# cmavro/GNN-RAG

Measured on NVIDIA H100. Metric: questions/sec (GNN forward+score) on WebQSP-shape subgraphs; agg-kernel HBM GB/s, higher is better.
Workload: dtype f32

## Files before the change

### gnn_rag_b200/csrc/linear_tc.cu

```cuda
#include "wgmma.cuh"

namespace gr {

int g_tc_cluster = 1;
int g_tc_bk = 32;
int g_tc_tma_store = 1;

namespace {

using namespace tc;
constexpr int kThreads = 384;
constexpr int kConsumerWarps = 8;
constexpr int kLaunchRegs = 168, kProducerRegs = 40, kConsumerRegs = 232;
static_assert(128 * kProducerRegs + 256 * kConsumerRegs <= kThreads * kLaunchRegs, "register budget");

__global__ void split_bf16_seg_kernel(const float* __restrict__ W, int64_t ldw, int64_t N, int64_t Kpad,
                                      int seg, int pitch, __nv_bfloat16* __restrict__ hi,
                                      __nv_bfloat16* __restrict__ lo, int64_t ldo) {
  const int64_t total = N * Kpad;
  const int64_t stride = (int64_t)gridDim.x * blockDim.x;
  for (int64_t i = (int64_t)blockIdx.x * blockDim.x + threadIdx.x; i < total; i += stride) {
    const int64_t n = i / Kpad, k = i - n * Kpad;
    const int sidx = (int)(k / pitch), c = (int)(k - (int64_t)sidx * pitch);
    float v = c < seg ? __ldg(W + n * ldw + (int64_t)sidx * seg + c) : 0.f;
// ... 14 lines not shown
    float v[4] = {0.f, 0.f, 0.f, 0.f};
    const float* src = A + m * lda + k;
    if (vec_ok && k + 3 < K) {
      float4 t = __ldg(reinterpret_cast<const float4*>(src));
      v[0] = t.x; v[1] = t.y; v[2] = t.z; v[3] = t.w;
    } else {
#pragma unroll
      for (int q = 0; q < 4; ++q)
        if (k + q < K) v[q] = __ldg(src + q);
    }
    __nv_bfloat16 h[4], l[4];
#pragma unroll
    for (int q = 0; q < 4; ++q) {
      h[q] = __float2bfloat16_rn(v[q]);
      l[q] = __float2bfloat16_rn(v[q] - __bfloat162float(h[q]));
    }
    __nv_bfloat16* ph = hi + m * ldo + k;
    __nv_bfloat16* pl = lo + m * ldo + k;
    if (vec_st && k + 3 < ldo) {
      *reinterpret_cast<uint2*>(ph) = *reinterpret_cast<uint2*>(h);
      *reinterpret_cast<uint2*>(pl) = *reinterpret_cast<uint2*>(l);
    } else {
#pragma unroll
      for (int q = 0; q < 4; ++q)
        if (k + q < ldo) { ph[q] = h[q]; pl[q] = l[q]; }
    }
  }
}

struct TcParams {
  const float* bias;
  float* C;
  int64_t ldc;
  __nv_bfloat16* c_hi;
  __nv_bfloat16* c_lo;
  int64_t ldc16;
  const float* w_score;
  float* dots;
  int M, N, K, n_pad, n16, stages, num_tiles;
  uint32_t flags;
  int tma_store;
  int kg_T, kg_G, kg_pitch, kg_nkb, kg_one0, kg_one1, kg_nb0;
};

template <int NP, int CS, int BK, bool GROUPED>
__global__ void __launch_bounds__(kThreads, 1)
linear_tc_kernel(const __grid_constant__ CUtensorMap map_a_hi, const __grid_constant__ CUtensorMap map_a_lo,
                 const __grid_constant__ CUtensorMap map_w_hi, const __grid_constant__ CUtensorMap map_w_lo,
                 const __grid_constant__ CUtensorMap map_c, const __grid_constant__ CUtensorMap map_c_hi,
                 const __grid_constant__ CUtensorMap map_c_lo, const TcParams p) {
  extern __shared__ __align__(1024) uint8_t smem_raw[];
  uint8_t* smem = reinterpret_cast<uint8_t*>((reinterpret_cast<uintptr_t>(smem_raw) + 1023) & ~(uintptr_t)1023);
  const int a_bytes = BM * BK * 2;
  constexpr int w_bytes = NP * BK * 2;
  const bool single = (p.flags & GR_LINEAR_BF16_SINGLE) != 0;
  const int w_off = single ? a_bytes : 2 * a_bytes;
  const int stage_bytes = single ? a_bytes + w_bytes : 2 * a_bytes + 2 * w_bytes;
  uint8_t* s_out = smem + (size_t)p.stages * stage_bytes;
  uint64_t* bars = reinterpret_cast<uint64_t*>(s_out + 2 * kStageOutBytes);
  uint64_t* full_bar = bars;
  uint64_t* empty_bar = bars + p.stages;
  float* s_bias = reinterpret_cast<float*>(bars + 2 * p.stages);
  float* s_ws = s_bias + 256;
  for (int i = threadIdx.x; i < 256; i += kThreads) {
    s_bias[i] = (p.bias && i < p.N) ? p.bias[i] : 0.f;
    s_ws[i] = (p.w_score && i < p.N) ? p.w_score[i] : 0.f;
// ... 67 lines not shown
    const bool vec_h = p.c_hi && (p.ldc16 % 2 == 0) && ((reinterpret_cast<uintptr_t>(p.c_hi) & 3) == 0) &&
                       ((reinterpret_cast<uintptr_t>(p.c_lo) & 3) == 0);
    uint32_t phase = 0;
    int s = 0;
    for (int g = cid; g < ngroups; g += ncluster) {
      const int tile = g * CS + crank;
      float acc[NP / 2];
#pragma unroll
      for (int i = 0; i < NP / 2; ++i) acc[i] = 0.f;
      int prev = -1;
      for (int kb = 0; kb < nkb; ++kb) {
        mbar_wait(&full_bar[s], phase);
        const uint32_t sa = smem_u32(smem + (size_t)s * stage_bytes);
        const uint32_t a_row = (uint32_t)(cw * WG_M * BK * 2);
        const uint64_t da_hi = make_smem_desc<BK>(sa + a_row), da_lo = make_smem_desc<BK>(sa + a_bytes + a_row);
        const uint64_t dw_hi = make_smem_desc<BK>(sa + w_off), dw_lo = make_smem_desc<BK>(sa + w_off + w_bytes);
        if constexpr (GROUPED) {
          if (kb >= p.kg_one0 && kb < p.kg_one1) mma_kblock<NP, BK, 1, false>(acc, da_hi, da_lo, dw_hi, dw_lo);
          else mma_kblock<NP, BK, BK / MMA_K, false>(acc, da_hi, da_lo, dw_hi, dw_lo);
        } else if (single) {
          mma_kblock<NP, BK, BK / MMA_K, true>(acc, da_hi, da_lo, dw_hi, dw_lo);
        } else {
          mma_kblock<NP, BK, BK / MMA_K, false>(acc, da_hi, da_lo, dw_hi, dw_lo);
        }
        wgmma_wait<1>();
        if (prev >= 0 && lane == 0) release_slot<CS>(&empty_bar[prev]);
        prev = s;
        if (++s == p.stages) { s = 0; phase ^= 1; }
      }
      wgmma_wait<0>();
      if (prev >= 0 && lane == 0) release_slot<CS>(&empty_bar[prev]);

      const int64_t row0 = (int64_t)tile * BM + cw * WG_M + r;
      float dot0 = 0.f, dot1 = 0.f;
#pragma unroll
      for (int q = 0; q < NP / 16; ++q) {
        const int c0 = 16 * q;
        if (c0 >= p.n_pad) continue;
        float v[8];
        epi_values(acc, q, cq, e, v, dot0, dot1);
        if (p.tma_store) {
          epi_store_tma(v, stg, r, cq, issuer, 1 + cw, &map_c, &map_c_hi, &map_c_lo, p.C != nullptr,
                        p.c_hi != nullptr, c0, tile * BM + cw * WG_M);
          continue;
        }
#pragma unroll
        for (int b = 0; b < 2; ++b) {
          const int col = c0 + 8 * b + 2 * cq;
#pragma unroll
          for (int hr = 0; hr < 2; ++hr) {
            const int64_t row = row0 + 8 * hr;
            if (row >= p.M) continue;
            const float x0 = v[4 * b + 2 * hr], x1 = v[4 * b + 2 * hr + 1];
            if (p.C) {
              float* c = p.C + row * p.ldc + col;
              if (vec_c && col + 1 < p.N) {
                *reinterpret_cast<float2*>(c) = make_float2(x0, x1);
              } else {
                if (col < p.N) c[0] = x0;
                if (col + 1 < p.N) c[1] = x1;
              }
            }
            if (p.c_hi) {
              uint32_t lo;
              const uint32_t hi = split_hi_lo(x0, x1, lo);
              unsigned short* ph = reinterpret_cast<unsigned short*>(p.c_hi + row * p.ldc16 + col);
              unsigned short* pl = reinterpret_cast<unsigned short*>(p.c_lo + row * p.ldc16 + col);
              if (vec_h && col + 1 < p.n16) {
                *reinterpret_cast<uint32_t*>(ph) = hi;
                *reinterpret_cast<uint32_t*>(pl) = lo;
              } else {
                if (col < p.n16) { ph[0] = (unsigned short)(hi & 0xFFFF); pl[0] = (unsigned short)(lo & 0xFFFF); }
                if (col + 1 < p.n16) { ph[1] = (unsigned short)(hi >> 16); pl[1] = (unsigned short)(lo >> 16); }
              }
            }
          }
        }
      }
      epi_dots(dot0, dot1, p.dots, row0, p.M, cq);
    }
    if (p.tma_store && issuer) asm volatile("cp.async.bulk.wait_group 0;" ::: "memory");
  }
  __syncthreads();
  if (CS > 1) cluster_sync_all();
}

struct TcPlan {
  int64_t kp;
  int n_pad, np, stages, bk;
  size_t a_plane_bytes, w_plane_bytes, total_bytes, w_only_bytes, smem_bytes;
  bool ok;
};

TcPlan plan_tc(int64_t M, int64_t N, int64_t K, bool single = false) {
  TcPlan t{};
  const int BK = g_tc_bk == 64 ? 64 : 32;
// ... 117 lines not shown
                            void* workspace, size_t workspace_bytes, void* stream_) {
  using namespace gr;
  cudaStream_t stream = reinterpret_cast<cudaStream_t>(stream_);
  GR_CHECK_ARG(A && W && C && workspace, "null pointer");
  GR_CHECK_ARG(M > 0 && N > 0 && K > 0, "M, N, K must be positive");
  GR_CHECK_ARG(lda >= K && ldw >= K && ldc >= N, "leading dimension smaller than row length");
  GR_CHECK_ARG(M < (int64_t)0x7fffffff - BM, "M exceeds int32 range");
  TcPlan t = plan_tc(M, N, K);
  if (!t.ok) {
    set_error("gr_linear_tc: unsupported shape M=%lld N=%lld K=%lld (need 8 <= N <= 256, K >= 8)",
              (long long)M, (long long)N, (long long)K);
    return GR_ERR_UNSUPPORTED;
  }
  if (int rc = check_workspace(__func__, workspace, workspace_bytes, t.total_bytes)) return rc;
  if ((reinterpret_cast<uintptr_t>(workspace) & 255) != 0) {
    set_error("gr_linear_tc: workspace must be 256-byte aligned");
    return GR_ERR_INVALID_ARG;
  }
  char* ws = reinterpret_cast<char*>(workspace);
  __nv_bfloat16* a_hi = reinterpret_cast<__nv_bfloat16*>(ws);
  __nv_bfloat16* a_lo = reinterpret_cast<__nv_bfloat16*>(ws + t.a_plane_bytes);
  __nv_bfloat16* w_hi = reinterpret_cast<__nv_bfloat16*>(ws + 2 * t.a_plane_bytes);
  __nv_bfloat16* w_lo = reinterpret_cast<__nv_bfloat16*>(ws + 2 * t.a_plane_bytes + t.w_plane_bytes);
  int rc = split_launch(A, lda, M, K, a_hi, a_lo, t.kp, stream);
  if (rc != GR_OK) return rc;
  rc = split_launch(W, ldw, N, K, w_hi, w_lo, t.kp, stream);
  if (rc != GR_OK) return rc;
  TcParams p{};
  p.bias = bias; p.C = C; p.ldc = ldc;
  p.M = (int)M; p.N = (int)N; p.K = (int)K; p.flags = flags;
  return launch_tc(a_hi, a_lo, t.kp, w_hi, w_lo, t.kp, t, p, stream);
}

extern "C" int gr_linear_tc_planes(const void* A_hi, const void* A_lo, int64_t lda16, const float* W,
                                   int64_t ldw, const float* bias, float* C, int64_t ldc, void* C_hi,
                                   void* C_lo, int64_t ldc16, const float* w_score, float* dots, int64_t M,
                                   int64_t N, int64_t K, int64_t k_seg, int64_t k_seg_pitch, uint32_t flags,
                                   void* workspace, size_t workspace_bytes, void* stream_) {
  using namespace gr;
  cudaStream_t stream = reinterpret_cast<cudaStream_t>(stream_);
  GR_CHECK_ARG(A_hi && (A_lo || (flags & GR_LINEAR_BF16_SINGLE)) && W && workspace, "null pointer");
  GR_CHECK_ARG(C || C_hi, "no output requested");
  GR_CHECK_ARG(M > 0 && N > 0 && K > 0, "M, N, K must be positive");
  const bool grouped = (flags & GR_LINEAR_K_GROUPED) != 0;
  const bool korder = (flags & GR_LINEAR_K_ORDER_PLANES) != 0;
  GR_CHECK_ARG(!korder || grouped, "GR_LINEAR_K_ORDER_PLANES modifies GR_LINEAR_K_GROUPED and needs it");
  if (grouped) {
    GR_CHECK_ARG(k_seg > 0 && k_seg_pitch >= k_seg && k_seg_pitch % 16 == 0,
                 "GR_LINEAR_K_GROUPED needs segmented K: k_seg > 0 and k_seg_pitch >= k_seg, a multiple of 16");
    GR_CHECK_ARG(K % k_seg_pitch == 0 && (K / k_seg_pitch) % 2 == 1,
                 "GR_LINEAR_K_GROUPED needs an odd number of segments (2 I + 1)");
    GR_CHECK_ARG(g_tc_bk != 64, "GR_LINEAR_K_GROUPED needs 32-column k-blocks (tc_bk = 32)");
    GR_CHECK_ARG(!(flags & GR_LINEAR_BF16_SINGLE), "GR_LINEAR_K_GROUPED does not combine with GR_LINEAR_BF16_SINGLE");
  }
  const bool segmented = grouped || (k_seg > 0 && k_seg_pitch > k_seg);
  GR_CHECK_ARG(lda16 >= K && lda16 % 8 == 0, "lda16 must be >= K and a multiple of 8");
  GR_CHECK_ARG(!segmented || K % k_seg_pitch == 0, "K must be a multiple of k_seg_pitch");
  GR_CHECK_ARG(ldw >= (segmented ? K / k_seg_pitch * k_seg : K), "ldw smaller than the weight row length");
  GR_CHECK_ARG(!C || ldc >= N, "ldc smaller than N");
  GR_CHECK_ARG(!C_hi || (C_lo && ldc16 >= N), "C_lo missing or ldc16 smaller than N");
  GR_CHECK_ARG(!dots || w_score, "dots requested without w_score");
  GR_CHECK_ARG(M < (int64_t)0x7fffffff - BM, "M exceeds int32 range");
  TcPlan t = plan_tc(M, N, K, (flags & GR_LINEAR_BF16_SINGLE) != 0);
  if (!t.ok) {
    set_error("gr_linear_tc_planes: unsupported shape M=%lld N=%lld K=%lld", (long long)M, (long long)N,
              (long long)K);
    return GR_ERR_UNSUPPORTED;
  }
  const int num_ins = grouped ? (int)(K / k_seg_pitch / 2) : 0;
  const GroupedK gk = grouped ? plan_grouped_k(k_seg_pitch, num_ins, N, korder) : GroupedK{};
  const int64_t nb0 = (k_seg_pitch + 31) / 32 * 32;
  GR_CHECK_ARG(!korder || lda16 >= nb0 + 2 * num_ins * k_seg_pitch,
               "GR_LINEAR_K_ORDER_PLANES: lda16 must cover the neighbour region (round32(k_seg_pitch) + (K - k_seg_pitch) "
               "columns)");
  const size_t w_plane_bytes = grouped ? gk.w_plane_bytes : t.w_plane_bytes;
  if (workspace_bytes < 2 * w_plane_bytes || (reinterpret_cast<uintptr_t>(workspace) & 255) != 0) {
    set_error("gr_linear_tc_planes: workspace too small or not 256-byte aligned");
    return GR_ERR_WORKSPACE;
  }
  char* ws = reinterpret_cast<char*>(workspace);
  __nv_bfloat16* w_hi = reinterpret_cast<__nv_bfloat16*>(ws);
  __nv_bfloat16* w_lo = reinterpret_cast<__nv_bfloat16*>(ws + w_plane_bytes);
  int rc = GR_OK;
  if (flags & GR_LINEAR_W_PRESPLIT) {
  } else if (grouped) {
    rc = grouped_w_split(W, ldw, N, (int)k_seg, num_ins, gk, w_hi, w_lo, stream);
  } else if (segmented) {
    int64_t work = N * K;
    int grid = (int)std::min<int64_t>(ceil_div(work, 256), 32LL * sm_count());
    split_bf16_seg_kernel<<<grid, 256, 0, stream>>>(W, ldw, N, K, (int)k_seg, (int)k_seg_pitch, w_hi, w_lo, t.kp);
    GR_CHECK_LAUNCH();
  } else {
    rc = split_launch(W, ldw, N, K, w_hi, w_lo, t.kp, stream);
  }
  if (rc != GR_OK) return rc;
  TcParams p{};
  p.bias = bias; p.C = C; p.ldc = ldc;
  p.c_hi = reinterpret_cast<__nv_bfloat16*>(C_hi); p.c_lo = reinterpret_cast<__nv_bfloat16*>(C_lo);
  p.ldc16 = ldc16; p.w_score = w_score; p.dots = dots;
  p.M = (int)M; p.N = (int)N; p.K = (int)K; p.flags = flags;
  if (grouped) {
    p.kg_T = 2 * num_ins + 1; p.kg_pitch = (int)k_seg_pitch; p.kg_nkb = gk.nkb;
    const bool tail = gk.ksteps_last == 1;
    if (!korder) {
      p.kg_G = gk.G;
      p.kg_one0 = tail ? (gk.G - 1) * p.kg_T : gk.nkb; p.kg_one1 = gk.nkb;
    } else {
      p.kg_G = tail ? gk.G - 1 : gk.G; p.kg_nb0 = (int)nb0;
      p.kg_one0 = tail ? p.kg_G * p.kg_T : gk.nkb; p.kg_one1 = tail ? p.kg_one0 + 1 : gk.nkb;
    }
  }
  return launch_tc(reinterpret_cast<const __nv_bfloat16*>(A_hi),
                   reinterpret_cast<const __nv_bfloat16*>(A_lo ? A_lo : A_hi), lda16, w_hi, w_lo,
                   grouped ? gk.kp : t.kp, t, p, stream);
}
```

### gnn_rag_b200/models.py

```python
import numpy as np
import torch
import torch.nn as nn
import torch.nn.functional as F

from . import autograd_path, batching, ops
from .modules import (AttnEncoder, BERTInstruction, Fusion, GraftLayer, LSTMInstruction, NSMLayer, QueryReform,
                      ReasonGNNLayer, TypeLayer)

VERY_SMALL_NUMBER = 1e-10


def _no_autocast():
    return torch.autocast("cuda", enabled=False)


class BaseModel(nn.Module):
    def __init__(self, args, num_entity, num_relation, num_word):
        super().__init__()
        self.num_relation, self.num_entity, self.num_word = num_relation, num_entity, num_word
        self.kge_frozen = args["kge_frozen"]
        self.kg_dim = args["kg_dim"]
        self.entity_emb_file = args["entity_emb_file"]
        self.relation_emb_file = args["relation_emb_file"]
        self.relation_word_emb = args["relation_word_emb"]
# ... 182 lines not shown
            return ops.rel_features_from_embeddings(
                [self.relation_embedding.weight, self.relation_embedding_inv.weight], lin.weight, lin.bias)
        rel, rel_inv = self.get_rel_feature_train()
        return ops.rel_features_from_tensors([rel.contiguous(), rel_inv.contiguous()])

    def get_rel_feature_train(self):
        if self.rel_texts is None:
            lin = self.relation_linear
            return lin(self.relation_embedding.weight), lin(self.relation_embedding_inv.weight)
        return (self._rel_text_features(self.rel_features, self.rel_texts, self.self_att_r),
                self._rel_text_features(self.rel_features_inv, self.rel_texts, self.self_att_r))

    def forward(self, batch, training=False):
        if training:
            return autograd_path.rearev_forward(self, batch)
        with torch.no_grad(), _no_autocast():
            return self._forward_infer(batch)

    def _forward_infer(self, batch):
        dev = self._check_ready()
        D, I = self.entity_dim, self.num_ins
        db = batching.stage_batch(batch, dev, self.num_relation + 1, self.normalized_gnn, self.norm_rel)
        self.last_batch = db
        B, N = db.B, db.N
        instructions = self._fork_instructions(db.q_input)
        rel_f = self.get_rel_feature()
        self.reasoning.init_reason(db, rel_f)
        self._get_ent_init(db, rel_f, self.reasoning)
        instructions = self._join_instructions(instructions)
        self.dist_history = [db.seed_dist]
        h = None
        reforms = [getattr(self, "reform" + str(j)).fusion for j in range(I)]
        Wr, Wg = [f.r.weight for f in reforms], [f.g.weight for f in reforms]
        for _t in range(self.num_iter):
            relation_ins = instructions
            dist = db.seed_dist
            for j in range(self.num_gnn):
                dist, hj = self.reasoning(dist, relation_ins, step=j, need_h=(j == self.num_gnn - 1),
                                          sparse_prior=(j == 0))
                h = hj if hj is not None else h
            self.dist_history.append(dist)
            instructions = ops.query_reform(db.query_entities, h, instructions, Wr, Wg, B, N)
        pred_dist = self.dist_history[-1]
        loss, pred = self._loss_and_pred(pred_dist, db.answer_dist)
        return loss, pred, pred_dist, None


class NSM(BaseModel):
    def __init__(self, args, num_entity, num_relation, num_word):
        super().__init__(args, num_entity, num_relation, num_word)
        D = self.entity_dim
        self.num_step = args["num_step"]
        self.num_iter = self.num_step
        self.model_name = args["model_name"].lower()
        self.lambda_constrain, self.lambda_back = args["lambda_constrain"], args["lambda_back"]
        if self.lambda_back != 0.0 or self.lambda_constrain != 0.0:
            raise NotImplementedError("NSM backward-consistency branch is broken in the reference "
                                      "(nsm_gnn.py:122 reads an unset attribute); not reproduced")
        self.linear_dropout = args["linear_dropout"]
        self.entity_linear = nn.Linear(self.ent_dim, D)
        self.relation_linear1 = nn.Linear(self.rel_dim, D)
        self.relation_linear2 = nn.Linear(self.rel_dim, D)
        self.kg_lin = nn.Linear(D, D)
        self.score_func = nn.Linear(2 * D, 1)
        self.linear_drop = nn.Dropout(p=self.linear_dropout)
        if self.encode_type:
            self.type_layer = TypeLayer(D, D, self.linear_drop, self.device, self.norm_rel)
        self.self_att_r = AttnEncoder(D)
        self.self_att_r2 = AttnEncoder(D)
        self.reasoning = NSMLayer(args, num_entity, num_relation, D)
        self.reasoning2 = NSMLayer(args, num_entity, num_relation, D)
        self.instruction = self._make_instruction(args)
        self.to(self.device)

    def get_rel_feature(self):
# ... 117 lines not shown
```

### gnn_rag_b200/modules.py

```python
import torch
import torch.nn as nn
import torch.nn.functional as F

from . import ops

VERY_NEG_NUMBER = -100000000000


class TypeLayer(nn.Module):

    def __init__(self, in_features, out_features, linear_drop, device, norm_rel):
        super().__init__()
        self.in_features, self.out_features = in_features, out_features
        self.linear_drop = linear_drop
        self.kb_self_linear = nn.Linear(in_features, out_features)
        self.device = device
        self.norm_rel = norm_rel

    def forward(self, graph, rel_features, out, planes=None):
        table = ops.rel_table(rel_features, self.kb_self_linear.weight, self.kb_self_linear.bias, dirs=1)[0]
        wt, wh = (graph.wr_t, graph.wr_h) if self.norm_rel else (None, None)
        ops.type_layer(graph, table, out, wt, wh, planes=planes)
        return out

# ... 221 lines not shown
        if self.use_planes:
            self.Dp = (D + 15) // 16 * 16
            self.Kpad = Kd // D * self.Dp
            Kp = (self.Kpad + 63) // 64 * 64
            key = (str(device), Nt, Kp, D)
            if key not in _GraphLayerBase._plane_cache:
                _GraphLayerBase._plane_cache.clear()
                _GraphLayerBase._plane_cache[key] = [
                    [torch.zeros(Nt, Kp, dtype=torch.bfloat16, device=device) for _ in range(2)]
                    for _ in range(2)]
            self.P = _GraphLayerBase._plane_cache[key]
            self.h32 = torch.empty(Nt, D, dtype=torch.float32, device=device)
            self.h32_valid = False
            self.fr_rows = torch.empty(Nt, dtype=torch.int32, device=device)
            self.fr_count = torch.zeros(1, dtype=torch.int32, device=device)
            self.dots = torch.empty(2 * Nt, dtype=torch.float32, device=device)
        else:
            self.X = [torch.empty(Nt, Kd, dtype=torch.float32, device=device) for _ in range(2)]

    @property
    def h_view(self):
        if not self.use_planes:
            return self.X[self.cur][:, : self.entity_dim]
        if not self.h32_valid:
            D = self.entity_dim
            hi, lo = self.P[self.cur]
            torch.add(hi[:, :D].float(), lo[:, :D].float(), out=self.h32)
            self.h32_valid = True
        return self.h32

    def cur_planes(self):
        return tuple(self.P[self.cur]) if self.use_planes else None

    def _e2e_and_score(self, e2e, mask, need_h32=True):
        D = self.entity_dim
        sw, sb = self.score_func.weight.view(-1), self.score_func.bias
        if self.use_planes:
            hi, lo = self.P[self.cur]
            nhi, nlo = self.P[1 - self.cur]
            ops.linear_tc_planes(hi, lo, self.Kpad, e2e.weight, e2e.bias, out=self.h32 if need_h32 else None,
                                 out_planes=(nhi, nlo), w_score=sw, dots=self.dots, relu=True, k_seg=D,
                                 k_seg_pitch=self.Dp, single_ok=True)
            self.h32_valid = bool(need_h32)
            self.cur = 1 - self.cur
            return ops.masked_softmax(self.dots, sb, mask, self.B, self.N)
        X, Xn = self.X[self.cur], self.X[1 - self.cur]
        ops.e2e_linear(X, e2e.weight, e2e.bias, Xn[:, :D])
        self.cur = 1 - self.cur
        return ops.score_softmax(self.h_view, sw, sb, mask, self.B, self.N)


class ReasonGNNLayer(_GraphLayerBase):
    def __init__(self, args, num_entity, num_relation, entity_dim, alg):
        super().__init__()
        assert alg == "bfs"
        self.num_entity, self.num_relation, self.entity_dim = num_entity, num_relation, entity_dim
        self.num_ins, self.num_gnn = args["num_ins"], args["num_gnn"]
        self.use_posemb = args["pos_emb"]
        self.normalized_gnn = args["normalized_gnn"]
        D = entity_dim
        self.score_func = nn.Linear(D, 1)
        self.glob_lin = nn.Linear(D, D)
        self.lin = nn.Linear(2 * D, D)
        for i in range(self.num_gnn):
            self.add_module("rel_linear" + str(i), nn.Linear(D, D))
            self.add_module("e2e_linear" + str(i), nn.Linear(2 * self.num_ins * D + D, D))
            if self.use_posemb:
                self.add_module("pos_emb" + str(i), nn.Embedding(num_relation, D))
                self.add_module("pos_emb_inv" + str(i), nn.Embedding(num_relation, D))
        self.lin_m = nn.Linear(self.num_ins * D, D)
        self.linear_drop_train = nn.Dropout(p=args.get("linear_dropout", 0.0))

    def init_reason(self, db, rel_features):
        D = self.entity_dim
        self.graph = db.graph
# ... 2 lines not shown
        self._alloc(db.B * db.N, (2 * self.num_ins + 1) * D, db.local_entity.device)
        self.tables = []
        for k in range(self.num_gnn):
            lin = getattr(self, "rel_linear" + str(k))
            add = None
            if self.use_posemb:
                add = [getattr(self, "pos_emb" + str(k)).weight, getattr(self, "pos_emb_inv" + str(k)).weight]
            tf, ti = ops.rel_table(rel_features, lin.weight, lin.bias, addends=add)
            pn = None
            if self.use_planes and ops.aggregate_dual_abs_supported(db.N, D, self.Dp, tf.shape[0]):
                pn_all = ops.pad_table256(tf._base if tf._base is not None else torch.cat([tf, ti]))
                pn = (pn_all[: tf.shape[0]], pn_all[tf.shape[0]:])
            self.tables.append((tf, ti, pn))

    def _forward_sparse_prior(self, current_dist, relational_ins, step, need_h):
        D = self.entity_dim
        g = self.graph
        tf, ti, _pn = self.tables[step]
        wt, wh = (g.w_t, g.w_h) if self.normalized_gnn else (None, None)
        e2e = getattr(self, "e2e_linear" + str(step))
        sw, sb = self.score_func.weight.view(-1), self.score_func.bias
        cur, nxt = tuple(self.P[self.cur]), tuple(self.P[1 - self.cur])
        ops.frontier_rows(g, current_dist, self.fr_rows, self.fr_count)
        ops.linear_tc_planes(cur[0], cur[1], self.Dp, e2e.weight[:, :D], e2e.bias,
                             out=self.h32 if need_h else None, out_planes=nxt, w_score=sw, dots=self.dots,
                             relu=True, k_seg=D, k_seg_pitch=self.Dp)
        ops.frontier_fixup(g, current_dist, tf, ti, relational_ins, cur, e2e.weight, e2e.bias, sw, nxt,
                           self.h32 if need_h else None, self.dots, self.fr_rows, self.fr_count, wt, wh)
        self.h32_valid = bool(need_h)
        self.cur = 1 - self.cur
        dist = ops.masked_softmax(self.dots, sb, self.local_entity_mask, self.B, self.N)
        return dist, (self.h_view if need_h else None)

    def forward(self, current_dist, relational_ins, step=0, need_h=True, sparse_prior=False):
        D = self.entity_dim
        g = self.graph
        if sparse_prior and self.use_planes and ops.SPARSE_PRIOR_FASTPATH:
            return self._forward_sparse_prior(current_dist, relational_ins, step, need_h)
        tf, ti, pn = self.tables[step]
        wt, wh = (g.w_t, g.w_h) if self.normalized_gnn else (None, None)
        e2e = getattr(self, "e2e_linear" + str(step))
        if (self.use_planes and pn is not None and ops.AGG_ABS and ops.FUSED_LAYER and not ops.ACT_BF16
                and self.B * self.N >= ops.FUSED_MIN_ROWS and ops.fused_layer_supported(self.N, D, self.Dp, self.num_ins, D)):
            sw, sb = self.score_func.weight.view(-1), self.score_func.bias
            ops.dense_layer(g, current_dist, pn[0], pn[1], relational_ins, self.cur_planes(), self.Dp, e2e.weight,
                            e2e.bias, out=self.h32 if need_h else None, out_planes=tuple(self.P[1 - self.cur]),
                            w_score=sw, dots=self.dots, w_t=wt, w_h=wh)
            self.h32_valid = bool(need_h)
            self.cur = 1 - self.cur
            dist = ops.masked_softmax(self.dots, sb, self.local_entity_mask, self.B, self.N)
            return dist, (self.h_view if need_h else None)
        if self.use_planes and pn is not None and ops.AGG_ABS:
            ops.aggregate_dual_abs(g, current_dist, pn[0], pn[1], relational_ins, self.cur_planes(), self.Dp,
                                  self.Dp, wt, wh)
        elif self.use_planes:
            ops.aggregate_dual(g, current_dist, tf, ti, relational_ins, None, self.Dp, wt, wh,
                               planes=self.cur_planes(), seg_pitch=self.Dp)
        else:
            ops.aggregate_dual(g, current_dist, tf, ti, relational_ins, self.X[self.cur], D, wt, wh)
        dist = self._e2e_and_score(getattr(self, "e2e_linear" + str(step)), self.local_entity_mask, need_h)
        return dist, (self.h_view if need_h else None)


class NSMLayer(_GraphLayerBase):
    def __init__(self, args, num_entity, num_relation, entity_dim):
        super().__init__()
        self.num_entity, self.num_relation, self.entity_dim = num_entity, num_relation, entity_dim
        self.num_steps = args["num_step"]
        self.reason_kb = args["reason_kb"]
        self.normalized_gnn = args["normalized_gnn"]
        D = entity_dim
        self.score_func = nn.Linear(D, 1)
        self.lin = nn.Linear(2 * D, D)
        for i in range(self.num_steps):
            self.add_module("rel_linear" + str(i), nn.Linear(D, D))
            self.add_module("e2e_linear" + str(i), nn.Linear(2 * D, D))
        self.linear_drop_train = nn.Dropout(p=args.get("linear_dropout", 0.0))

    def init_reason(self, db, rel_features):
        D = self.entity_dim
        self.graph = db.graph
        self.B, self.N = db.B, db.N
        self.local_entity_mask = (db.local_entity != self.num_entity).float().view(-1)
        self._alloc(db.B * db.N, 2 * D, db.local_entity.device)
        self.tables = []
        for k in range(self.num_steps):
            lin = getattr(self, "rel_linear" + str(k))
            self.tables.append(ops.rel_table(rel_features, lin.weight, lin.bias, dirs=1)[0])
        self.possible = torch.empty(db.B * db.N, dtype=torch.float32, device=db.local_entity.device)
        if self.use_planes:
            self.nb32 = torch.empty(db.B * db.N, D, dtype=torch.float32, device=db.local_entity.device)

    def forward(self, current_dist, relational_ins, step=0):
        D = self.entity_dim
# ... 120 lines not shown
```

### gnn_rag_b200/ops.py

```python
import contextlib
import ctypes
import functools
import weakref

import numpy as np
import torch

from . import _lib

LINEAR_RELU = 1
LINEAR_EXACT_FP32 = 2
LINEAR_W_PRESPLIT = 4
LINEAR_BF16_SINGLE = 8
LINEAR_K_GROUPED = 16
LINEAR_K_ORDER_PLANES = 32
AGG_K_ORDER = 1

ACT_BF16 = False


class _Stats:

    def __init__(self):
        self.launches = 0
# ... 342 lines not shown
        ell, nbytes = _workspace(g.rowptr_t.device, "gr_fused_ell_bytes", g.B, g.N, g.F)
        _launch("gr_fused_ell_build", _p(g.rowptr_t), _p(g.src_t), _p(g.rel_t), _p(w_t),
                _p(g.rowptr_h), _p(g.src_h), _p(g.rel_h), _p(w_h), g.B, g.N, g.F, _p(ell), nbytes, op="csr_build")
        setattr(g, key, ell)
    return ell


def fused_layer(g, prior, pn_fwd, pn_inv, ins, h_planes, seg_pitch, W, bias, out=None, out_planes=None,
                w_score=None, dots=None, relu=True, w_t=None, w_h=None):
    prior = _cuda(prior, torch.float32, "prior").contiguous()
    ins = _cuda(ins, torch.float32, "ins").contiguous()
    B, I, D = ins.shape
    hi, lo = h_planes
    n_out = W.shape[0]
    assert pn_fwd.is_contiguous() and pn_inv.is_contiguous() and hi.stride(0) == lo.stride(0)
    assert W.stride(1) == 1 and W.shape[1] == (2 * I + 1) * D
    nbytes = _L().gr_fused_layer_workspace_bytes(D, seg_pitch, I, n_out)
    ws, presplit = _weight_ws(W, n_out, W.shape[1], "fused", seg_pitch, nbytes)
    ell = fused_ell(g, w_t, w_h)
    chi, clo = out_planes if out_planes is not None else (None, None)
    flags = (LINEAR_RELU if relu else 0) | (LINEAR_W_PRESPLIT if presplit else 0)
    _launch("gr_fused_layer", _p(g.rowptr_t), _p(g.src_t), _p(g.rel_t), _p(w_t),
            _p(g.rowptr_h), _p(g.src_h), _p(g.rel_h), _p(w_h),
            _p(prior), _p(pn_fwd), _p(pn_inv), _p(ins), _p(hi), _p(lo), hi.stride(0), seg_pitch,
            _p(W), W.stride(0), _p(bias), _p(out), out.stride(0) if out is not None else 0,
            _p(chi), _p(clo), chi.stride(0) if chi is not None else 0, _p(w_score), _p(dots),
            B, g.N, D, I, n_out, g.F, flags, _p(ws), ws.numel(), _p(ell), ell.numel(),
            launches=2 if (w_t is not None or w_h is not None) else 1,
            op="fused_layer")
    return out


def dense_layer(g, prior, pn_fwd, pn_inv, ins, planes, seg_pitch, W, bias, out=None, out_planes=None, w_score=None,
                dots=None, w_t=None, w_h=None):
    I, n_out = ins.shape[1], W.shape[0]
    if DENSE_WIDE_AS_PAIR and (n_out + 15) // 16 * 16 > 128:
        aggregate_dual_abs(g, prior, pn_fwd, pn_inv, ins, planes, k_order_nb0(seg_pitch), seg_pitch, w_t, w_h,
                           k_order=True)
        return linear_tc_planes(planes[0], planes[1], (2 * I + 1) * seg_pitch, W, bias, out=out, out_planes=out_planes,
                                w_score=w_score, dots=dots, relu=True, k_seg=ins.shape[2], k_seg_pitch=seg_pitch,
                                k_grouped=True, k_order=True)
    return fused_layer(g, prior, pn_fwd, pn_inv, ins, planes, seg_pitch, W, bias, out=out, out_planes=out_planes,
                       w_score=w_score, dots=dots, relu=True, w_t=w_t, w_h=w_h)


def type_layer(g, table, out, w_t=None, w_h=None, planes=None):
    table = _cuda(table, torch.float32, "table").contiguous()
    D = table.shape[1]
    io = _node_io(out=out)
    assert out is None or out.stride(1) == 1
    hi, lo = planes if planes is not None else (None, None)
    _launch("gr_type_layer", _p(g.rowptr_t), _p(g.rel_t), _p(w_t), _p(g.rowptr_h), _p(g.rel_h), _p(w_h), _p(table),
            _p(out), out.stride(0) if out is not None else 0, _p(hi), _p(lo), hi.stride(0) if hi is not None else 0,
            g.B, g.N, D, g.F, io=io, op="type_layer")
    return out


def split_bf16(A, hi, lo):
    A = _cuda(A, torch.float32, "A")
    M, K = A.shape
    assert A.stride(1) == 1 and hi.stride(1) == 1 and hi.stride(0) == lo.stride(0)
    _launch("gr_split_bf16", _p(A), A.stride(0), M, K, _p(hi), _p(lo), hi.stride(0))


WEIGHT_CACHE = True
_CACHE = {}
_PRIVATE = None


@contextlib.contextmanager
def graph_private_weights():
    global _PRIVATE
    prev, _PRIVATE = _PRIVATE, []
    try:
# ... 25 lines not shown
            for k in [k for k, e in _CACHE.items() if e[2]() is None]:
                del _CACHE[k]
        _CACHE[key] = [buffers, owner._version, weakref.ref(owner)]
    return buffers, False


def _weight_ws(W, N, K, k_seg, k_seg_pitch, nbytes):
    (ws,), presplit = _cached(("ws", W.data_ptr(), W.stride(0), N, K, k_seg, k_seg_pitch), _base(W),
                              lambda b: b[0].numel() >= nbytes,
                              lambda: (torch.empty(nbytes, dtype=torch.uint8, device=W.device),))
    return ws, presplit


def param_planes(P):
    M, K = P.shape
    Kp = (K + 63) // 64 * 64
    (hi, lo), current = _cached(("planes", P.data_ptr()), P, lambda b: b[0].shape[0] == M,
                                lambda: tuple(torch.zeros(M, Kp, dtype=torch.bfloat16, device=P.device)
                                              for _ in range(2)))
    if not current:
        split_bf16(P.detach(), hi, lo)
    return hi, lo


def clear_weight_cache():
    _CACHE.clear()


def live_weight_workspaces():
    return [t for e in _CACHE.values() for t in e[0]]


def linear_tc_planes(a_hi, a_lo, K, W, bias, out=None, out_planes=None, w_score=None, dots=None, relu=True,
                     k_seg=0, k_seg_pitch=0, single_ok=False, k_grouped=False, k_order=False):
    N = W.shape[0]
    if N > TC_MAX_N:
        nsl = (N + TC_MAX_N - 1) // TC_MAX_N
        step = ((N + nsl - 1) // nsl + 15) // 16 * 16
        part = None
        for n0 in range(0, N, step):
            n1 = min(N, n0 + step)
            d = torch.empty_like(dots) if (dots is not None and n0 > 0) else dots
            linear_tc_planes(a_hi, a_lo, K, W[n0:n1], None if bias is None else bias[n0:n1],
                             out=None if out is None else out[:, n0:n1],
                             out_planes=None if out_planes is None else (out_planes[0][:, n0:n1], out_planes[1][:, n0:n1]),
                             w_score=None if w_score is None else w_score[n0:n1], dots=d, relu=relu, k_seg=k_seg,
                             k_seg_pitch=k_seg_pitch, single_ok=single_ok, k_grouped=k_grouped, k_order=k_order)
            if dots is not None and n0 > 0:
                part = d if part is None else part + d
        if part is not None:
            dots += part
        return out
    M = a_hi.shape[0]
    assert a_hi.dtype == torch.bfloat16 and a_hi.stride(1) == 1 and a_hi.stride(0) == a_lo.stride(0)
    if k_seg and k_seg_pitch > k_seg:
        assert K % k_seg_pitch == 0 and W.shape[1] == K // k_seg_pitch * k_seg
    else:
        assert W.shape[1] == K
    assert W.stride(1) == 1
    assert k_grouped or not k_order
    if k_grouped:
        nbytes = _L().gr_fused_layer_workspace_bytes(k_seg, k_seg_pitch, K // k_seg_pitch // 2, N)
        ws, presplit = _weight_ws(W, N, W.shape[1], "korder" if k_order else "fused", k_seg_pitch, nbytes)
    else:
        nbytes = _L().gr_linear_tc_planes_workspace_bytes(N, K)
        ws, presplit = _weight_ws(W, N, K, k_seg, k_seg_pitch, nbytes)
    chi, clo = out_planes if out_planes is not None else (None, None)
    flags = (LINEAR_RELU if relu else 0) | (LINEAR_W_PRESPLIT if presplit else 0) | \
        (LINEAR_K_GROUPED if k_grouped else LINEAR_BF16_SINGLE if (ACT_BF16 and single_ok) else 0) | \
        (LINEAR_K_ORDER_PLANES if k_order else 0)
    _launch("gr_linear_tc_planes", _p(a_hi), _p(a_lo), a_hi.stride(0), _p(W), W.stride(0), _p(bias),
            _p(out), out.stride(0) if out is not None else 0,
            _p(chi), _p(clo), chi.stride(0) if chi is not None else 0,
            _p(w_score), _p(dots), M, N, K, k_seg, k_seg_pitch, flags, _p(ws), nbytes,
            launches=1 if presplit else 2, op="gemm_tc", info=(M, N, K))
    return out


class RelFeatures:

    _buf = {}

    def __init__(self, R1, D, n_dir, device, planes):
        self.R1, self.D, self.n_dir = R1, D, n_dir
        self.hi = self.lo = self.f32 = None
        if planes:
            Kp = (D + 63) // 64 * 64
            key = (str(device), n_dir * R1, Kp)
            if key not in RelFeatures._buf:
                RelFeatures._buf[key] = (torch.zeros(n_dir * R1, Kp, dtype=torch.bfloat16, device=device),
                                         torch.zeros(n_dir * R1, Kp, dtype=torch.bfloat16, device=device))
            self.hi, self.lo = RelFeatures._buf[key]
        else:
            self.f32 = torch.empty(n_dir * R1, D, dtype=torch.float32, device=device)

    def rows(self, d):
        return slice(d * self.R1, (d + 1) * self.R1)


def rel_features_from_embeddings(embs, W, bias):
    R1, K = embs[0].shape
    D = W.shape[0]
    planes = tc_planes_ok(D, K) and tc_planes_ok(D, D)
    rf = RelFeatures(R1, D, len(embs), W.device, planes)
    for d, E in enumerate(embs):
        if planes:
            ahi, alo = param_planes(E)
# ... 922 lines not shown
```

### include/gnnrag_b200.h

```cpp
#ifndef GNNRAG_B200_H_
#define GNNRAG_B200_H_

#include <stddef.h>
#include <stdint.h>

#ifdef __cplusplus
extern "C" {
#endif

#define GR_ABI_VERSION 1

typedef enum gr_status {
  GR_OK = 0,
  GR_ERR_INVALID_ARG = -1,
  GR_ERR_CUDA = -2,
  GR_ERR_WORKSPACE = -3,
  GR_ERR_UNSUPPORTED = -4
} gr_status;

#define GR_LINEAR_RELU 1u
#define GR_LINEAR_EXACT_FP32 2u
#define GR_LINEAR_BF16_SINGLE 8u
#define GR_LINEAR_W_PRESPLIT 4u

#define GR_LINEAR_K_GROUPED 16u
#define GR_LINEAR_K_ORDER_PLANES 32u

int gr_abi_version(void);
const char* gr_last_error(void);
int gr_set_option(const char* name, int64_t value);
static inline int64_t gr_pad4(int64_t n) { return (n + 3) & ~(int64_t)3; }

size_t gr_csr_build_workspace_bytes(int64_t F, int64_t Nt);
int gr_csr_build(const void* heads, const void* rels, const void* tails, int idx_bytes,
                 int64_t F, int64_t Nt, int64_t num_rel_rows,
                 int32_t* rowptr_t, int32_t* src_t, int32_t* rel_t, int32_t* fact_t,
                 int32_t* rowptr_h, int32_t* src_h, int32_t* rel_h, int32_t* fact_h,
                 int32_t* status, const int32_t* nfacts, void* workspace, size_t workspace_bytes, void* stream);

int gr_gather_f32(const float* in, const int32_t* fact, float* out, int64_t F, void* stream);

int gr_linear(const float* A, int64_t lda, const float* W, int64_t ldw, const float* bias,
              const float* addend, int64_t ld_addend, int64_t addend_rows,
              float* C, int64_t ldc, int64_t M, int64_t N, int64_t K, uint32_t flags, void* stream);

size_t gr_linear_tc_workspace_bytes(int64_t M, int64_t N, int64_t K);
int gr_linear_tc(const float* A, int64_t lda, const float* W, int64_t ldw, const float* bias,
                 float* C, int64_t ldc, int64_t M, int64_t N, int64_t K, uint32_t flags,
                 void* workspace, size_t workspace_bytes, void* stream);
size_t gr_linear_tc_planes_workspace_bytes(int64_t N, int64_t K);
int gr_linear_tc_planes(const void* A_hi, const void* A_lo, int64_t lda16, const float* W, int64_t ldw,
                        const float* bias, float* C, int64_t ldc, void* C_hi, void* C_lo, int64_t ldc16,
                        const float* w_score, float* dots, int64_t M, int64_t N, int64_t K,
                        int64_t k_seg, int64_t k_seg_pitch,
                        uint32_t flags, void* workspace, size_t workspace_bytes, void* stream);
int gr_split_bf16(const float* A, int64_t lda, int64_t M, int64_t K, void* hi, void* lo, int64_t ld_out,
                  void* stream);

int gr_aggregate(const int32_t* rowptr, const int32_t* src, const int32_t* rel, const float* w,
                 const float* prior, const float* table, const float* ins,
                 float* out, int64_t out_row_stride, int64_t out_col0, int64_t seg_stride,
                 float* possible, int B, int N, int D, int I, int64_t F, void* stream);

int gr_aggregate_backward(const int32_t* rowptr, const int32_t* src, const int32_t* rel, const float* w,
                          const float* prior, const float* table, const float* ins, const float* grad_out,
                          int64_t grad_row_stride, int64_t grad_col0, int64_t seg_stride, float* grad_table,
                          float* grad_ins, float* grad_prior, int B, int N, int D, int I, int64_t F, void* stream);

int gr_aggregate_dual(const int32_t* rowptr_t, const int32_t* src_t, const int32_t* rel_t,
                      const float* w_t, const int32_t* rowptr_h, const int32_t* src_h,
                      const int32_t* rel_h, const float* w_h, const float* prior,
                      const float* table_fwd, const float* table_inv, const float* ins,
                      float* out, int64_t out_row_stride, int64_t out_col0, int64_t seg_pitch,
                      void* out_hi, void* out_lo, int64_t ld_planes,
                      int B, int N, int D, int I, int64_t F, void* stream);

int gr_pad_table256(const float* table, int64_t ldt, int64_t rows, int D, float* pn, void* stream);
int gr_aggregate_dual_abs_supported(int N, int D, int64_t seg_pitch, int64_t R1);
int gr_aggregate_dual_abs(const int32_t* rowptr_t, const int32_t* src_t, const int32_t* rel_t, const float* w_t,
                         const int32_t* rowptr_h, const int32_t* src_h, const int32_t* rel_h, const float* w_h,
                         const float* prior, const float* pn_fwd, const float* pn_inv, int64_t table_rows,
                         const float* ins, void* out_hi, void* out_lo, int64_t ld_planes, int64_t out_col0,
                         int64_t seg_pitch, int B, int N, int D, int I, int64_t F, int32_t* tile_counter, void* stream);
#define GR_AGG_K_ORDER 1u
int gr_aggregate_dual_abs_ex(const int32_t* rowptr_t, const int32_t* src_t, const int32_t* rel_t, const float* w_t,
                             const int32_t* rowptr_h, const int32_t* src_h, const int32_t* rel_h, const float* w_h,
                             const float* prior, const float* pn_fwd, const float* pn_inv, int64_t table_rows,
                             const float* ins, void* out_hi, void* out_lo, int64_t ld_planes, int64_t out_col0,
// ... 328 lines not shown
```

Before: 12970.

## Skip unused outputs: seed-row-only fp32 h, no next planes or reform on final iteration

Adds a row-predicate variant of the planes GEMM that writes fp32 C only for rows flagged nonzero (the query/seed entities). The query-reform step only reads h at those rows. The final layer of the final iteration also skips writing the bf16 next-layer planes, and the last iteration skips query_reform entirely, whose result was unused. This removes most fp32 output stores and some plane writes. The cost is a per-row predicate load and a non-TMA store path when rows are masked.

```diff
diff --git a/gnn_rag_b200/csrc/linear_tc.cu b/gnn_rag_b200/csrc/linear_tc.cu
--- a/gnn_rag_b200/csrc/linear_tc.cu
+++ b/gnn_rag_b200/csrc/linear_tc.cu
@@ -70,6 +70,7 @@
   const float* bias;
   float* C;
   int64_t ldc;
+  const float* c_rows;
   __nv_bfloat16* c_hi;
   __nv_bfloat16* c_lo;
   int64_t ldc16;
@@ -203,6 +204,11 @@
       if (prev >= 0 && lane == 0) release_slot<CS>(&empty_bar[prev]);
 
       const int64_t row0 = (int64_t)tile * BM + cw * WG_M + r;
+      bool keep[2] = {true, true};
+      if (p.c_rows) {
+        keep[0] = row0 < p.M && p.c_rows[row0] != 0.f;
+        keep[1] = row0 + 8 < p.M && p.c_rows[row0 + 8] != 0.f;
+      }
       float dot0 = 0.f, dot1 = 0.f;
 #pragma unroll
       for (int q = 0; q < NP / 16; ++q) {
@@ -211,9 +217,9 @@
         float v[8];
         epi_values(acc, q, cq, e, v, dot0, dot1);
         if (p.tma_store) {
-          epi_store_tma(v, stg, r, cq, issuer, 1 + cw, &map_c, &map_c_hi, &map_c_lo, p.C != nullptr,
+          epi_store_tma(v, stg, r, cq, issuer, 1 + cw, &map_c, &map_c_hi, &map_c_lo, p.C && !p.c_rows,
                         p.c_hi != nullptr, c0, tile * BM + cw * WG_M);
-          continue;
+          if (!p.c_rows) continue;
         }
 #pragma unroll
         for (int b = 0; b < 2; ++b) {
@@ -223,7 +229,7 @@
             const int64_t row = row0 + 8 * hr;
             if (row >= p.M) continue;
             const float x0 = v[4 * b + 2 * hr], x1 = v[4 * b + 2 * hr + 1];
-            if (p.C) {
+            if (p.C && keep[hr]) {
               float* c = p.C + row * p.ldc + col;
               if (vec_c && col + 1 < p.N) {
                 *reinterpret_cast<float2*>(c) = make_float2(x0, x1);
@@ -232,7 +238,7 @@
                 if (col + 1 < p.N) c[1] = x1;
               }
             }
-            if (p.c_hi) {
+            if (p.c_hi && !p.tma_store) {
               uint32_t lo;
               const uint32_t hi = split_hi_lo(x0, x1, lo);
               unsigned short* ph = reinterpret_cast<unsigned short*>(p.c_hi + row * p.ldc16 + col);
@@ -416,50 +422,52 @@
   return launch_tc(a_hi, a_lo, t.kp, w_hi, w_lo, t.kp, t, p, stream);
 }
 
-extern "C" int gr_linear_tc_planes(const void* A_hi, const void* A_lo, int64_t lda16, const float* W,
-                                   int64_t ldw, const float* bias, float* C, int64_t ldc, void* C_hi,
-                                   void* C_lo, int64_t ldc16, const float* w_score, float* dots, int64_t M,
-                                   int64_t N, int64_t K, int64_t k_seg, int64_t k_seg_pitch, uint32_t flags,
-                                   void* workspace, size_t workspace_bytes, void* stream_) {
-  using namespace gr;
-  cudaStream_t stream = reinterpret_cast<cudaStream_t>(stream_);
-  GR_CHECK_ARG(A_hi && (A_lo || (flags & GR_LINEAR_BF16_SINGLE)) && W && workspace, "null pointer");
-  GR_CHECK_ARG(C || C_hi, "no output requested");
-  GR_CHECK_ARG(M > 0 && N > 0 && K > 0, "M, N, K must be positive");
+namespace gr {
+namespace {
+
+int linear_tc_planes_entry(const char* fn, const void* A_hi, const void* A_lo, int64_t lda16, const float* W,
+                           int64_t ldw, const float* bias, float* C, int64_t ldc, const float* c_rows, void* C_hi,
+                           void* C_lo, int64_t ldc16, const float* w_score, float* dots, int64_t M, int64_t N,
+                           int64_t K, int64_t k_seg, int64_t k_seg_pitch, uint32_t flags, void* workspace,
+                           size_t workspace_bytes, cudaStream_t stream) {
+  GR_CHECK_ARG_AS(fn, A_hi && (A_lo || (flags & GR_LINEAR_BF16_SINGLE)) && W && workspace, "null pointer");
+  GR_CHECK_ARG_AS(fn, C || C_hi, "no output requested");
+  GR_CHECK_ARG_AS(fn, !c_rows || C, "c_rows selects rows of C and needs C");
+  GR_CHECK_ARG_AS(fn, M > 0 && N > 0 && K > 0, "M, N, K must be positive");
   const bool grouped = (flags & GR_LINEAR_K_GROUPED) != 0;
   const bool korder = (flags & GR_LINEAR_K_ORDER_PLANES) != 0;
-  GR_CHECK_ARG(!korder || grouped, "GR_LINEAR_K_ORDER_PLANES modifies GR_LINEAR_K_GROUPED and needs it");
+  GR_CHECK_ARG_AS(fn, !korder || grouped, "GR_LINEAR_K_ORDER_PLANES modifies GR_LINEAR_K_GROUPED and needs it");
   if (grouped) {
-    GR_CHECK_ARG(k_seg > 0 && k_seg_pitch >= k_seg && k_seg_pitch % 16 == 0,
-                 "GR_LINEAR_K_GROUPED needs segmented K: k_seg > 0 and k_seg_pitch >= k_seg, a multiple of 16");
-    GR_CHECK_ARG(K % k_seg_pitch == 0 && (K / k_seg_pitch) % 2 == 1,
-                 "GR_LINEAR_K_GROUPED needs an odd number of segments (2 I + 1)");
-    GR_CHECK_ARG(g_tc_bk != 64, "GR_LINEAR_K_GROUPED needs 32-column k-blocks (tc_bk = 32)");
-    GR_CHECK_ARG(!(flags & GR_LINEAR_BF16_SINGLE), "GR_LINEAR_K_GROUPED does not combine with GR_LINEAR_BF16_SINGLE");
+    GR_CHECK_ARG_AS(fn, k_seg > 0 && k_seg_pitch >= k_seg && k_seg_pitch % 16 == 0,
+                    "GR_LINEAR_K_GROUPED needs segmented K: k_seg > 0 and k_seg_pitch >= k_seg, a multiple of 16");
+    GR_CHECK_ARG_AS(fn, K % k_seg_pitch == 0 && (K / k_seg_pitch) % 2 == 1,
+                    "GR_LINEAR_K_GROUPED needs an odd number of segments (2 I + 1)");
+    GR_CHECK_ARG_AS(fn, g_tc_bk != 64, "GR_LINEAR_K_GROUPED needs 32-column k-blocks (tc_bk = 32)");
+    GR_CHECK_ARG_AS(fn, !(flags & GR_LINEAR_BF16_SINGLE),
+                    "GR_LINEAR_K_GROUPED does not combine with GR_LINEAR_BF16_SINGLE");
   }
   const bool segmented = grouped || (k_seg > 0 && k_seg_pitch > k_seg);
-  GR_CHECK_ARG(lda16 >= K && lda16 % 8 == 0, "lda16 must be >= K and a multiple of 8");
-  GR_CHECK_ARG(!segmented || K % k_seg_pitch == 0, "K must be a multiple of k_seg_pitch");
-  GR_CHECK_ARG(ldw >= (segmented ? K / k_seg_pitch * k_seg : K), "ldw smaller than the weight row length");
-  GR_CHECK_ARG(!C || ldc >= N, "ldc smaller than N");
-  GR_CHECK_ARG(!C_hi || (C_lo && ldc16 >= N), "C_lo missing or ldc16 smaller than N");
-  GR_CHECK_ARG(!dots || w_score, "dots requested without w_score");
-  GR_CHECK_ARG(M < (int64_t)0x7fffffff - BM, "M exceeds int32 range");
+  GR_CHECK_ARG_AS(fn, lda16 >= K && lda16 % 8 == 0, "lda16 must be >= K and a multiple of 8");
+  GR_CHECK_ARG_AS(fn, !segmented || K % k_seg_pitch == 0, "K must be a multiple of k_seg_pitch");
+  GR_CHECK_ARG_AS(fn, ldw >= (segmented ? K / k_seg_pitch * k_seg : K), "ldw smaller than the weight row length");
+  GR_CHECK_ARG_AS(fn, !C || ldc >= N, "ldc smaller than N");
+  GR_CHECK_ARG_AS(fn, !C_hi || (C_lo && ldc16 >= N), "C_lo missing or ldc16 smaller than N");
+  GR_CHECK_ARG_AS(fn, !dots || w_score, "dots requested without w_score");
+  GR_CHECK_ARG_AS(fn, M < (int64_t)0x7fffffff - BM, "M exceeds int32 range");
   TcPlan t = plan_tc(M, N, K, (flags & GR_LINEAR_BF16_SINGLE) != 0);
   if (!t.ok) {
-    set_error("gr_linear_tc_planes: unsupported shape M=%lld N=%lld K=%lld", (long long)M, (long long)N,
-              (long long)K);
+    set_error("%s: unsupported shape M=%lld N=%lld K=%lld", fn, (long long)M, (long long)N, (long long)K);
     return GR_ERR_UNSUPPORTED;
   }
   const int num_ins = grouped ? (int)(K / k_seg_pitch / 2) : 0;
   const GroupedK gk = grouped ? plan_grouped_k(k_seg_pitch, num_ins, N, korder) : GroupedK{};
   const int64_t nb0 = (k_seg_pitch + 31) / 32 * 32;
-  GR_CHECK_ARG(!korder || lda16 >= nb0 + 2 * num_ins * k_seg_pitch,
-               "GR_LINEAR_K_ORDER_PLANES: lda16 must cover the neighbour region (round32(k_seg_pitch) + (K - k_seg_pitch) "
-               "columns)");
+  GR_CHECK_ARG_AS(fn, !korder || lda16 >= nb0 + 2 * num_ins * k_seg_pitch,
+                  "GR_LINEAR_K_ORDER_PLANES: lda16 must cover the neighbour region (round32(k_seg_pitch) + "
+                  "(K - k_seg_pitch) columns)");
   const size_t w_plane_bytes = grouped ? gk.w_plane_bytes : t.w_plane_bytes;
   if (workspace_bytes < 2 * w_plane_bytes || (reinterpret_cast<uintptr_t>(workspace) & 255) != 0) {
-    set_error("gr_linear_tc_planes: workspace too small or not 256-byte aligned");
+    set_error("%s: workspace too small or not 256-byte aligned", fn);
     return GR_ERR_WORKSPACE;
   }
   char* ws = reinterpret_cast<char*>(workspace);
@@ -479,7 +487,7 @@
   }
   if (rc != GR_OK) return rc;
   TcParams p{};
-  p.bias = bias; p.C = C; p.ldc = ldc;
+  p.bias = bias; p.C = C; p.ldc = ldc; p.c_rows = c_rows;
   p.c_hi = reinterpret_cast<__nv_bfloat16*>(C_hi); p.c_lo = reinterpret_cast<__nv_bfloat16*>(C_lo);
   p.ldc16 = ldc16; p.w_score = w_score; p.dots = dots;
   p.M = (int)M; p.N = (int)N; p.K = (int)K; p.flags = flags;
@@ -498,3 +506,27 @@
                    reinterpret_cast<const __nv_bfloat16*>(A_lo ? A_lo : A_hi), lda16, w_hi, w_lo,
                    grouped ? gk.kp : t.kp, t, p, stream);
 }
+
+}
+}
+
+extern "C" int gr_linear_tc_planes(const void* A_hi, const void* A_lo, int64_t lda16, const float* W,
+                                   int64_t ldw, const float* bias, float* C, int64_t ldc, void* C_hi,
+                                   void* C_lo, int64_t ldc16, const float* w_score, float* dots, int64_t M,
+                                   int64_t N, int64_t K, int64_t k_seg, int64_t k_seg_pitch, uint32_t flags,
+                                   void* workspace, size_t workspace_bytes, void* stream) {
+  return gr::linear_tc_planes_entry(__func__, A_hi, A_lo, lda16, W, ldw, bias, C, ldc, nullptr, C_hi, C_lo, ldc16,
+                                    w_score, dots, M, N, K, k_seg, k_seg_pitch, flags, workspace, workspace_bytes,
+                                    reinterpret_cast<cudaStream_t>(stream));
+}
+
+extern "C" int gr_linear_tc_planes_rows(const void* A_hi, const void* A_lo, int64_t lda16, const float* W,
+                                        int64_t ldw, const float* bias, float* C, int64_t ldc, void* C_hi,
+                                        void* C_lo, int64_t ldc16, const float* w_score, float* dots, int64_t M,
+                                        int64_t N, int64_t K, int64_t k_seg, int64_t k_seg_pitch, uint32_t flags,
+                                        void* workspace, size_t workspace_bytes, const float* c_rows,
+                                        void* stream) {
+  return gr::linear_tc_planes_entry(__func__, A_hi, A_lo, lda16, W, ldw, bias, C, ldc, c_rows, C_hi, C_lo, ldc16,
+                                    w_score, dots, M, N, K, k_seg, k_seg_pitch, flags, workspace, workspace_bytes,
+                                    reinterpret_cast<cudaStream_t>(stream));
+}
diff --git a/gnn_rag_b200/models.py b/gnn_rag_b200/models.py
--- a/gnn_rag_b200/models.py
+++ b/gnn_rag_b200/models.py
@@ -238,15 +238,20 @@
         h = None
         reforms = [getattr(self, "reform" + str(j)).fusion for j in range(I)]
         Wr, Wg = [f.r.weight for f in reforms], [f.g.weight for f in reforms]
-        for _t in range(self.num_iter):
+        seed_rows = db.query_entities.reshape(-1)
+        for t in range(self.num_iter):
+            last_iter = t == self.num_iter - 1
             relation_ins = instructions
             dist = db.seed_dist
             for j in range(self.num_gnn):
-                dist, hj = self.reasoning(dist, relation_ins, step=j, need_h=(j == self.num_gnn - 1),
-                                          sparse_prior=(j == 0))
+                last = j == self.num_gnn - 1
+                dist, hj = self.reasoning(dist, relation_ins, step=j, need_h=last, sparse_prior=(j == 0),
+                                          h_rows=seed_rows if last and not last_iter else None,
+                                          next_layer=not (last and last_iter))
                 h = hj if hj is not None else h
             self.dist_history.append(dist)
-            instructions = ops.query_reform(db.query_entities, h, instructions, Wr, Wg, B, N)
+            if not last_iter:
+                instructions = ops.query_reform(db.query_entities, h, instructions, Wr, Wg, B, N)
         pred_dist = self.dist_history[-1]
         loss, pred = self._loss_and_pred(pred_dist, db.answer_dist)
         return loss, pred, pred_dist, None
diff --git a/gnn_rag_b200/modules.py b/gnn_rag_b200/modules.py
--- a/gnn_rag_b200/modules.py
+++ b/gnn_rag_b200/modules.py
@@ -277,15 +277,24 @@
     def cur_planes(self):
         return tuple(self.P[self.cur]) if self.use_planes else None
 
-    def _e2e_and_score(self, e2e, mask, need_h32=True):
+    def _next_planes(self, next_layer):
+        return tuple(self.P[1 - self.cur]) if next_layer else None
+
+    def _h_out(self, need_h, h_rows):
+        if not need_h:
+            return None
+        if h_rows is not None and self.use_planes and not self.h32_valid:
+            return self.h32
+        return self.h_view
+
+    def _e2e_and_score(self, e2e, mask, need_h32=True, next_layer=True):
         D = self.entity_dim
         sw, sb = self.score_func.weight.view(-1), self.score_func.bias
         if self.use_planes:
             hi, lo = self.P[self.cur]
-            nhi, nlo = self.P[1 - self.cur]
             ops.linear_tc_planes(hi, lo, self.Kpad, e2e.weight, e2e.bias, out=self.h32 if need_h32 else None,
-                                 out_planes=(nhi, nlo), w_score=sw, dots=self.dots, relu=True, k_seg=D,
-                                 k_seg_pitch=self.Dp, single_ok=True)
+                                 out_planes=self._next_planes(next_layer), w_score=sw, dots=self.dots, relu=True,
+                                 k_seg=D, k_seg_pitch=self.Dp, single_ok=True)
             self.h32_valid = bool(need_h32)
             self.cur = 1 - self.cur
             return ops.masked_softmax(self.dots, sb, mask, self.B, self.N)
@@ -354,7 +363,9 @@
         dist = ops.masked_softmax(self.dots, sb, self.local_entity_mask, self.B, self.N)
         return dist, (self.h_view if need_h else None)
 
-    def forward(self, current_dist, relational_ins, step=0, need_h=True, sparse_prior=False):
+    def forward(self, current_dist, relational_ins, step=0, need_h=True, sparse_prior=False, h_rows=None,
+                next_layer=True):
+        assert next_layer or (need_h and h_rows is None), "a last layer keeps the full fp32 h"
         D = self.entity_dim
         g = self.graph
         if sparse_prior and self.use_planes and ops.SPARSE_PRIOR_FASTPATH:
@@ -366,12 +377,12 @@
                 and self.B * self.N >= ops.FUSED_MIN_ROWS and ops.fused_layer_supported(self.N, D, self.Dp, self.num_ins, D)):
             sw, sb = self.score_func.weight.view(-1), self.score_func.bias
             ops.dense_layer(g, current_dist, pn[0], pn[1], relational_ins, self.cur_planes(), self.Dp, e2e.weight,
-                            e2e.bias, out=self.h32 if need_h else None, out_planes=tuple(self.P[1 - self.cur]),
-                            w_score=sw, dots=self.dots, w_t=wt, w_h=wh)
-            self.h32_valid = bool(need_h)
+                            e2e.bias, out=self.h32 if need_h else None, out_planes=self._next_planes(next_layer),
+                            w_score=sw, dots=self.dots, w_t=wt, w_h=wh, out_rows=h_rows if need_h else None)
+            self.h32_valid = bool(need_h) and h_rows is None
             self.cur = 1 - self.cur
             dist = ops.masked_softmax(self.dots, sb, self.local_entity_mask, self.B, self.N)
-            return dist, (self.h_view if need_h else None)
+            return dist, self._h_out(need_h, h_rows)
         if self.use_planes and pn is not None and ops.AGG_ABS:
             ops.aggregate_dual_abs(g, current_dist, pn[0], pn[1], relational_ins, self.cur_planes(), self.Dp,
                                   self.Dp, wt, wh)
@@ -380,8 +391,8 @@
                                planes=self.cur_planes(), seg_pitch=self.Dp)
         else:
             ops.aggregate_dual(g, current_dist, tf, ti, relational_ins, self.X[self.cur], D, wt, wh)
-        dist = self._e2e_and_score(getattr(self, "e2e_linear" + str(step)), self.local_entity_mask, need_h)
-        return dist, (self.h_view if need_h else None)
+        dist = self._e2e_and_score(getattr(self, "e2e_linear" + str(step)), self.local_entity_mask, need_h, next_layer)
+        return dist, self._h_out(need_h, h_rows)
 
 
 class NSMLayer(_GraphLayerBase):
diff --git a/gnn_rag_b200/ops.py b/gnn_rag_b200/ops.py
--- a/gnn_rag_b200/ops.py
+++ b/gnn_rag_b200/ops.py
@@ -398,14 +398,14 @@
 
 
 def dense_layer(g, prior, pn_fwd, pn_inv, ins, planes, seg_pitch, W, bias, out=None, out_planes=None, w_score=None,
-                dots=None, w_t=None, w_h=None):
+                dots=None, w_t=None, w_h=None, out_rows=None):
     I, n_out = ins.shape[1], W.shape[0]
     if DENSE_WIDE_AS_PAIR and (n_out + 15) // 16 * 16 > 128:
         aggregate_dual_abs(g, prior, pn_fwd, pn_inv, ins, planes, k_order_nb0(seg_pitch), seg_pitch, w_t, w_h,
                            k_order=True)
         return linear_tc_planes(planes[0], planes[1], (2 * I + 1) * seg_pitch, W, bias, out=out, out_planes=out_planes,
                                 w_score=w_score, dots=dots, relu=True, k_seg=ins.shape[2], k_seg_pitch=seg_pitch,
-                                k_grouped=True, k_order=True)
+                                k_grouped=True, k_order=True, **({} if out_rows is None else {"out_rows": out_rows}))
     return fused_layer(g, prior, pn_fwd, pn_inv, ins, planes, seg_pitch, W, bias, out=out, out_planes=out_planes,
                        w_score=w_score, dots=dots, relu=True, w_t=w_t, w_h=w_h)
 
@@ -497,7 +497,7 @@
 
 
 def linear_tc_planes(a_hi, a_lo, K, W, bias, out=None, out_planes=None, w_score=None, dots=None, relu=True,
-                     k_seg=0, k_seg_pitch=0, single_ok=False, k_grouped=False, k_order=False):
+                     k_seg=0, k_seg_pitch=0, single_ok=False, k_grouped=False, k_order=False, out_rows=None):
     N = W.shape[0]
     if N > TC_MAX_N:
         nsl = (N + TC_MAX_N - 1) // TC_MAX_N
@@ -510,7 +510,8 @@
                              out=None if out is None else out[:, n0:n1],
                              out_planes=None if out_planes is None else (out_planes[0][:, n0:n1], out_planes[1][:, n0:n1]),
                              w_score=None if w_score is None else w_score[n0:n1], dots=d, relu=relu, k_seg=k_seg,
-                             k_seg_pitch=k_seg_pitch, single_ok=single_ok, k_grouped=k_grouped, k_order=k_order)
+                             k_seg_pitch=k_seg_pitch, single_ok=single_ok, k_grouped=k_grouped, k_order=k_order,
+                             **({} if out_rows is None else {"out_rows": out_rows}))
             if dots is not None and n0 > 0:
                 part = d if part is None else part + d
         if part is not None:
@@ -531,13 +532,17 @@
         nbytes = _L().gr_linear_tc_planes_workspace_bytes(N, K)
         ws, presplit = _weight_ws(W, N, K, k_seg, k_seg_pitch, nbytes)
     chi, clo = out_planes if out_planes is not None else (None, None)
+    if out_rows is not None:
+        out_rows = _cuda(out_rows, torch.float32, "out_rows")
+        if out is None or not out_rows.is_contiguous() or out_rows.numel() != M:
+            raise ValueError("out_rows must be a contiguous fp32 [M] row predicate of out (M = %d)" % M)
     flags = (LINEAR_RELU if relu else 0) | (LINEAR_W_PRESPLIT if presplit else 0) | \
         (LINEAR_K_GROUPED if k_grouped else LINEAR_BF16_SINGLE if (ACT_BF16 and single_ok) else 0) | \
         (LINEAR_K_ORDER_PLANES if k_order else 0)
-    _launch("gr_linear_tc_planes", _p(a_hi), _p(a_lo), a_hi.stride(0), _p(W), W.stride(0), _p(bias),
+    _launch("gr_linear_tc_planes_rows", _p(a_hi), _p(a_lo), a_hi.stride(0), _p(W), W.stride(0), _p(bias),
             _p(out), out.stride(0) if out is not None else 0,
             _p(chi), _p(clo), chi.stride(0) if chi is not None else 0,
-            _p(w_score), _p(dots), M, N, K, k_seg, k_seg_pitch, flags, _p(ws), nbytes,
+            _p(w_score), _p(dots), M, N, K, k_seg, k_seg_pitch, flags, _p(ws), nbytes, _p(out_rows),
             launches=1 if presplit else 2, op="gemm_tc", info=(M, N, K))
     return out
 
diff --git a/include/gnnrag_b200.h b/include/gnnrag_b200.h
--- a/include/gnnrag_b200.h
+++ b/include/gnnrag_b200.h
@@ -54,6 +54,12 @@
                         const float* w_score, float* dots, int64_t M, int64_t N, int64_t K,
                         int64_t k_seg, int64_t k_seg_pitch,
                         uint32_t flags, void* workspace, size_t workspace_bytes, void* stream);
+int gr_linear_tc_planes_rows(const void* A_hi, const void* A_lo, int64_t lda16, const float* W, int64_t ldw,
+                             const float* bias, float* C, int64_t ldc, void* C_hi, void* C_lo, int64_t ldc16,
+                             const float* w_score, float* dots, int64_t M, int64_t N, int64_t K,
+                             int64_t k_seg, int64_t k_seg_pitch,
+                             uint32_t flags, void* workspace, size_t workspace_bytes, const float* c_rows,
+                             void* stream);
 int gr_split_bf16(const float* A, int64_t lda, int64_t M, int64_t K, void* hi, void* lo, int64_t ld_out,
                   void* stream);
 
```

Result: faster. 13570 (median of 6 runs) (+4.6%).
